# ebeauce/Seismic_BPMF

Measured on AMD Instinct MI355X. Metric: million network-CC-samples/s (matched filter), higher is better.
Workload: dtype f32

## Files before the change

### seismic_bpmf_amd/csrc/mf.hip

```cpp
#include "common.h"
#include "host_call.h"
#include "mf_split_api.h"
#include "mf_full_api.h"
#include <system_error>
#include <thread>
#include <chrono>
#include <vector>
#include <mutex>
#include <utility>
#include <cstring>
#include <algorithm>
#include "../../include/bpmf_hip.h"

#include <cstdlib>

namespace bpmf {

typedef float f32x16 __attribute__((ext_vector_type(16)));


__device__ __forceinline__ int2 mf_lag_range(bool any, long long mv_min, long long mv_max, long long step,
                                             long long L, long long N, long long n_corr, int exclusive_last)
{
    int2 r = make_int2(1, 0);
// ... 302 lines not shown
            mf_stage_rows<MAXR, MF_THREADS>(rd, rs_d, lag0 + mvc, tid);
            const __amdgpu_buffer_rsrc_t rs_t = __builtin_amdgcn_make_buffer_rsrc(
                (void*)(tmpl + ((size_t)t * n_ch + ch) * (size_t)L), 0, L * 4, 0x00020000);
            mf_stage_band<MAXT, MF_THREADS>(rt, rs_t, tid);
        };
        auto write_stage = [&](float* tp, float* dw) {
#pragma unroll
            for (int r = 0; r < MAXR; ++r) {
                const int x = tid + MF_THREADS * r;
                if (x < W) dw[mf_pad(x)] = rd[r];
            }
#pragma unroll
            for (int r = 0; r < MAXT; ++r) {
                const int x = tid + MF_THREADS * r;
                if (x < tp_len) tp[x] = rt[r];
            }
        };
        int4 rec = recs[0];
        int4 rec1 = recs[1];
        int ri = 0;
        if (rec.x >= 0) issue_stage(rec.x, rec.y);
        int buf = 0;
        while (rec.x >= 0) {
            const int ch = rec.x;
            float* tp = smem + buf * buf_floats;
            float* dw = tp + tp_len;
            write_stage(tp, dw);
            __syncthreads();
            const float w = __int_as_float(rec.z);
            const int mvc = rec.y;
            const float et = __int_as_float(rec.w);
            const int4 rec2 = recs[ri + 2];
            const float* edc = e_d + (size_t)ch * (size_t)nwin;
            f32x4 ed[4];
#pragma unroll
            for (int u = 0; u < 4; ++u) {
                const long long lag = lag_w + 256 * u;
                if (wg_inside || (lag + 3 >= rg.x && lag <= rg.y)) {
                    ed[u] = *(const f32x4u*)(edc + lag + mvc);
                } else {
                    ed[u] = (f32x4){0.0f, 0.0f, 0.0f, 0.0f};
                }
            }
            if (rec1.x >= 0) issue_stage(rec1.x, rec1.y);

            f32x4 acc[4];
#pragma unroll
            for (int u = 0; u < 4; ++u) acc[u] = (f32x4){0.0f, 0.0f, 0.0f, 0.0f};
            const int nq = Kpad >> 4;
            const unsigned a_addr = (unsigned)(size_t)(tp + a_base) ;
            const unsigned b_addr = (unsigned)(size_t)(dw + b_base);
            unsigned ap = a_addr, bp = b_addr;
            float sa[4], sb[4][4];
#define MF_LDS_READ(dst, addr, off) \
    asm volatile("ds_read_b32 %0, %1 offset:%2" : "=v"(dst) : "v"(addr), "n"(off))
#define MF_MFMA(slot, u) \
    acc[u] = __builtin_amdgcn_mfma_f32_16x16x4f32(sa[slot], sb[slot][u], acc[u], 0, 0, 0)
#define MF_REQ(slot, aoff, boff)                                    \
    MF_LDS_READ(sa[slot], ap, (aoff));                               \
    MF_LDS_READ(sb[slot][0], bp, (boff));                            \
    MF_LDS_READ(sb[slot][1], bp, (boff) + 1088);                     \
    MF_LDS_READ(sb[slot][2], bp, (boff) + 2176);                     \
    MF_LDS_READ(sb[slot][3], bp, (boff) + 3264)
#define MF_STEP(cur, req, aoff, boff)                                \
    asm volatile("s_waitcnt lgkmcnt(5)" ::: "memory");               \
    __builtin_amdgcn_sched_barrier(0);                               \
    MF_MFMA(cur, 0);                                                 \
    __builtin_amdgcn_sched_barrier(0);                               \
    MF_LDS_READ(sa[req], ap, (aoff));                                \
    __builtin_amdgcn_sched_barrier(0);                               \
    MF_MFMA(cur, 1);                                                 \
    __builtin_amdgcn_sched_barrier(0);                               \
    MF_LDS_READ(sb[req][0], bp, (boff));                             \
    __builtin_amdgcn_sched_barrier(0);                               \
    MF_MFMA(cur, 2);                                                 \
    __builtin_amdgcn_sched_barrier(0);                               \
    MF_LDS_READ(sb[req][1], bp, (boff) + 1088);                      \
    __builtin_amdgcn_sched_barrier(0);                               \
    MF_MFMA(cur, 3);                                                 \
    __builtin_amdgcn_sched_barrier(0);                               \
    MF_LDS_READ(sb[req][2], bp, (boff) + 2176);                      \
    MF_LDS_READ(sb[req][3], bp, (boff) + 3264);                      \
    __builtin_amdgcn_sched_barrier(0)
            __builtin_amdgcn_sched_barrier(0);
            if (prio) __builtin_amdgcn_s_setprio(0);
            MF_REQ(0, 0, 0);
            MF_REQ(1, 16, 16);
            for (int q = 0; q < nq; ++q) {
                MF_STEP(0, 2, 32, 32);
                MF_STEP(1, 3, 48, 48);
                MF_STEP(2, 0, 64, 68);
                MF_STEP(3, 1, 80, 84);
                ap += 64;
                bp += 68;
            }
            asm volatile("s_waitcnt lgkmcnt(0)" ::: "memory");
            __builtin_amdgcn_sched_barrier(0);
            if (prio == 1) __builtin_amdgcn_s_setprio(1);
            else if (prio == 2) __builtin_amdgcn_s_setprio(2);
            else if (prio == 3) __builtin_amdgcn_s_setprio(3);
#undef MF_LDS_READ
#undef MF_MFMA
#undef MF_REQ
#undef MF_STEP

            if (NETWORK_SUM && STEP1 && wg_inside) {
#pragma unroll
                for (int u = 0; u < 4; ++u) {
#pragma unroll
                    for (int r = 0; r < 4; ++r) {
                        const float cc = mf_cc_of<SQRT_NORM>(acc[u][r], et, ed[u][r]);
                        sum[u][r] = __fmaf_rn(w, cc, sum[u][r]);
                    }
                }
            } else {
#pragma unroll
            for (int u = 0; u < 4; ++u) {
#pragma unroll
                for (int r = 0; r < 4; ++r) {
                    const long long lag = lag_w + 256 * u + r;
                    const bool ok = lag >= rg.x && lag <= rg.y && (STEP1 || (unsigned)lag % (unsigned)step == 0);
                    float cc = 0.0f;
                    if (ok) {
                        cc = mf_cc_of<SQRT_NORM>(acc[u][r], et, ed[u][r]);
                        if (!NETWORK_SUM)
                            out[((size_t)t * n_corr + (STEP1 ? lag : (long long)((unsigned)lag / (unsigned)step))) * n_ch + ch] = cc;
                    }
                    if (NETWORK_SUM) sum[u][r] = __fmaf_rn(w, cc, sum[u][r]);
                }
            }
            }
            rec = rec1;
            rec1 = rec2;
            ++ri;
            buf ^= 1;
        }
    }
    if (NETWORK_SUM) {
#pragma unroll
        for (int u = 0; u < 4; ++u) {
            const long long lag = lag_w + 256 * u;
            float* dst = out + (size_t)t * n_corr + lag;
            if (STEP1 && lag + 3 < n_corr) {
                *(f32x4u*)dst = sum[u];
            } else {
#pragma unroll
                for (int r = 0; r < 4; ++r) {
                    const unsigned smp = (unsigned)(lag + r);
                    const long long i = STEP1 ? (long long)smp : (long long)(smp / (unsigned)step);
                    if ((STEP1 || smp % (unsigned)step == 0) && i < n_corr) out[(size_t)t * n_corr + i] = sum[u][r];
                }
            }
        }
    }
}

template <bool SQRT_NORM>
__device__ __forceinline__ int2 mf_fused_prologue(const float* __restrict__ tmpl, const int* __restrict__ mv,
                                                  const float* __restrict__ w, int t, int n_ch, long long step, int L,
                                                  long long N, long long n_corr, int exclusive_last,
                                                  int4* l_rec, int* l_part)
{
    const int tid = threadIdx.x, lane = tid & 63, wv = tid >> 6;
    float wc = 0.0f, nt = 0.0f;
    int m = 0;
    bool used = false;
    if (tid < n_ch) {
        wc = w[(size_t)t * n_ch + tid];
        used = !(wc == 0.0f);
    }
    const bool all_channels = (exclusive_last & 2) != 0;
    if (tid < n_ch && (used || all_channels)) m = mv[(size_t)t * n_ch + tid];
    if (used) {
        const float* x = tmpl + ((size_t)t * n_ch + tid) * (size_t)L;
        float acc = 0.0f;
        int l = 0;
        for (; l + 16 <= L; l += 16) {
            const f32x4u v0 = *(const f32x4u*)(x + l), v1 = *(const f32x4u*)(x + l + 4);
            const f32x4u v2 = *(const f32x4u*)(x + l + 8), v3 = *(const f32x4u*)(x + l + 12);
#pragma unroll
            for (int i = 0; i < 4; ++i) acc = __fmaf_rn(v0[i], v0[i], acc);
#pragma unroll
            for (int i = 0; i < 4; ++i) acc = __fmaf_rn(v1[i], v1[i], acc);
#pragma unroll
            for (int i = 0; i < 4; ++i) acc = __fmaf_rn(v2[i], v2[i], acc);
#pragma unroll
            for (int i = 0; i < 4; ++i) acc = __fmaf_rn(v3[i], v3[i], acc);
        }
        for (; l < L; ++l) acc = __fmaf_rn(x[l], x[l], acc);
        nt = SQRT_NORM ? acc : 1.0f / sqrtf(acc);
    }
    const unsigned long long mask = __ballot(used);
    const int idx = __popcll(mask & ((1ull << lane) - 1ull));
    const bool ranged = used || (all_channels && tid < n_ch);
    int mn = ranged ? m : 0x7fffffff, mx = ranged ? m : (int)0x80000000;
#pragma unroll
    for (int o = 32; o > 0; o >>= 1) {
        mn = min(mn, __shfl_xor(mn, o));
        mx = max(mx, __shfl_xor(mx, o));
    }
    if (lane == 0) {
        l_part[wv] = __popcll(mask);
        l_part[4 + wv] = mn;
        l_part[8 + wv] = mx;
    }
    __syncthreads();
    int base = 0, n_used = 0, mv_min_i = 0x7fffffff, mv_max_i = (int)0x80000000;
#pragma unroll
    for (int i = 0; i < 4; ++i) {
        const int c = l_part[i];
        if (i < wv) base += c;
        n_used += c;
        mv_min_i = min(mv_min_i, l_part[4 + i]);
        mv_max_i = max(mv_max_i, l_part[8 + i]);
    }
    if (used) l_rec[base + idx] = make_int4(tid, m, __float_as_int(wc), __float_as_int(nt));
    if (tid < MF_REC_TERMINATORS) l_rec[n_used + tid] = make_int4(-1, 0, 0, 0);
    __syncthreads();
    return mf_lag_range(n_used > 0, mv_min_i, mv_max_i, step, L, N, n_corr, exclusive_last);
}

#ifdef BPMF_PHASE_CYCLES
__device__ unsigned long long g_mf_phase[8];
#define MF_PHASE_DECL unsigned long long ph_last_ = 0, ph_acc_[4] = {0, 0, 0, 0}; unsigned ph_n_ = 0;
#define MF_PHASE_START() asm volatile("s_memtime %0\n\ts_waitcnt lgkmcnt(0)" : "=s"(ph_last_) :: "memory")
#define MF_PHASE(i)                                                                                \
    do {                                                                                           \
        unsigned long long t_;                                                                     \
        asm volatile("s_memtime %0\n\ts_waitcnt lgkmcnt(0)" : "=s"(t_) :: "memory");              \
        ph_acc_[i] += t_ - ph_last_;                                                               \
        ph_last_ = t_;                                                                             \
    } while (0)
#else
#define MF_PHASE_DECL
#define MF_PHASE_START() do {} while (0)
#define MF_PHASE(i) do {} while (0)
#endif

template <bool NETWORK_SUM, int MAXR, int MAXT, bool STEP1, int NTILE = 4, bool SQRT_NORM = false, bool FUSED = false, bool CSPLIT = false>
__global__ __launch_bounds__(MF_THREADS, 4) void mf_mfma_wave_kernel(
    const float* __restrict__ tmpl, const int4* __restrict__ chan_rec,
    const float* __restrict__ data, const float* __restrict__ e_d,
    const int2* __restrict__ range, int L, long long N, int T, int n_ch, long long n_corr, int step,
    float* __restrict__ out, int n_lag_blocks, int prio, const int* __restrict__ mv,
    const float* __restrict__ wts, int exclusive_last, int lag_block0)
{
    extern __shared__ float smem[];
    const int Kpad = mf_kpad(L);
    const int tp_len = mf_band_len(L);
    static_assert(NTILE == 4 || NTILE == 2 || NTILE == 1, "tiles per wave");
    static_assert(!CSPLIT || (NTILE == 1 && FUSED && NETWORK_SUM && STEP1), "channel split: the tiny-problem variant only");
    constexpr int LAGS_W = 256 * NTILE, LAGS_WG = CSPLIT ? LAGS_W : 4 * LAGS_W;
    constexpr int REC_STRIDE = CSPLIT ? 4 : 1;
    const int Ww = LAGS_W - 16 + Kpad;
    constexpr bool FULLW = NTILE < 4;
    const int Wbuf = FULLW ? 64 * MAXR : Ww;
    const int wave_floats = tp_len + (Wbuf + 2 * (Wbuf >> 4) + 2 + 63) / 64 * 64 + 64;

    const int tid = threadIdx.x;
    const int lane = tid & 63;
    const int wv = __builtin_amdgcn_readfirstlane(tid >> 6);
    const int a = lane & 15;
    const int kq = lane >> 4;

    int t;
    long long lag_block;
    if (!mf_tile_of_block(blockIdx.x, T, n_lag_blocks, t, lag_block)) return;
    lag_block += lag_block0;
    int2 rgi;
    int4* l_rec = nullptr;
    if constexpr (FUSED) {
        int* l_part = (int*)(smem + 4 * wave_floats + 64);
        l_rec = (int4*)(l_part + 16);
        const int2 r = mf_fused_prologue<SQRT_NORM>(tmpl, mv, wts, t, n_ch, (long long)step, L, N, n_corr, exclusive_last,
                                                    l_rec, l_part);
        rgi = make_int2(__builtin_amdgcn_readfirstlane(r.x), __builtin_amdgcn_readfirstlane(r.y));
    } else {
        rgi = range[t];
    }
    float* exch = nullptr;
    int n_used = 0;
    if constexpr (CSPLIT) {
        const int* l_part = (const int*)(smem + 4 * wave_floats + 64);
        n_used = l_part[0] + l_part[1] + l_part[2] + l_part[3];
        exch = (float*)(l_rec + n_ch + MF_REC_TERMINATORS);
    }
    const long long lag0 = lag_block * LAGS_WG + (CSPLIT ? 0 : (long long)wv * LAGS_W);
    const int2 rg = make_int2(rgi.x * step, rgi.y * step);
    const long long nwin = N - L + 1;

    f32x4 sum[NTILE];
#pragma unroll
    for (int u = 0; u < NTILE; ++u) sum[u] = (f32x4){0.0f, 0.0f, 0.0f, 0.0f};

    const bool wave_valid = rg.x <= rg.y && !(lag0 > rg.y || lag0 + LAGS_W - 1 < rg.x);
    const bool wave_inside = lag0 >= rg.x && lag0 + LAGS_W - 1 <= rg.y;
    const long long lag_w = lag0 + 16 * a + 4 * kq;
    MF_PHASE_DECL

    if (wave_valid) {
        float* tp = smem + wv * wave_floats;
        float* dw = tp + tp_len;
        const int a_base = 15 - a + kq;
        const int b_base = 18 * a + kq;
        const int4* __restrict__ recs = FUSED ? nullptr : chan_rec + (size_t)t * (n_ch + 2);
        auto ld_rec = [&](int i) -> int4 {
            if constexpr (FUSED) {
                const int4 v = l_rec[i];
                return make_int4(__builtin_amdgcn_readfirstlane(v.x), __builtin_amdgcn_readfirstlane(v.y),
                                 __builtin_amdgcn_readfirstlane(v.z), __builtin_amdgcn_readfirstlane(v.w));
            } else {
                return recs[i];
            }
        };

        float rd[MAXR], rt[MAXT];
        auto issue_stage = [&](int ch, int mvc) {
            const __amdgpu_buffer_rsrc_t rs_d = __builtin_amdgcn_make_buffer_rsrc(
                (void*)(data + (size_t)ch * (size_t)N), 0, (int)(N * 4), 0x00020000);
            mf_stage_rows<MAXR, 64>(rd, rs_d, lag0 + mvc, lane);
            const __amdgpu_buffer_rsrc_t rs_t = __builtin_amdgcn_make_buffer_rsrc(
                (void*)(tmpl + ((size_t)t * n_ch + ch) * (size_t)L), 0, L * 4, 0x00020000);
            mf_stage_band<MAXT, 64>(rt, rs_t, lane);
        };
        const int rd_chunks = (Ww + 63) >> 6, rt_chunks = (tp_len + 63) >> 6;
        auto write_stage = [&]() {
            if constexpr (FULLW) {
#pragma unroll
                for (int r = 0; r < MAXT; ++r) tp[lane + 64 * r] = rt[r];
#pragma unroll
                for (int r = 0; r < MAXR; ++r) {
                    const int x = lane + 64 * r;
                    dw[x + 2 * (x >> 4)] = rd[r];
                }
                return;
            }
#define MF_WT(r) case (r) + 1: if constexpr ((r) < MAXT) tp[lane + 64 * ((r) < MAXT ? (r) : 0)] = rt[(r) < MAXT ? (r) : 0]; [[fallthrough]];
            switch (rt_chunks) {
                MF_WT(4) MF_WT(3) MF_WT(2) MF_WT(1) MF_WT(0)
                default: break;
            }
#undef MF_WT
#define MF_WD(r) case (r) + 1: if constexpr ((r) < MAXR) { const int x = lane + 64 * (r); dw[x + 2 * (x >> 4)] = rd[(r) < MAXR ? (r) : 0]; } [[fallthrough]];
            switch (rd_chunks) {
                MF_WD(19) MF_WD(18) MF_WD(17) MF_WD(16) MF_WD(15) MF_WD(14) MF_WD(13) MF_WD(12) MF_WD(11) MF_WD(10)
                MF_WD(9) MF_WD(8) MF_WD(7) MF_WD(6) MF_WD(5) MF_WD(4) MF_WD(3) MF_WD(2) MF_WD(1) MF_WD(0)
                default: break;
            }
#undef MF_WD
        };

        int4 rec = ld_rec(CSPLIT ? wv : 0);
        int4 rec1 = ld_rec(CSPLIT ? wv + REC_STRIDE : 1);
        int ri = CSPLIT ? wv : 0;
        if (rec.x >= 0) issue_stage(rec.x, rec.y);
        MF_PHASE_START();
        while (rec.x >= 0) {
            const int ch = rec.x;
            write_stage();
            MF_PHASE(0);
            const float w = __int_as_float(rec.z);
            const int mvc = rec.y;
            const float et = __int_as_float(rec.w);
            const int4 rec2 = ld_rec(ri + 2 * REC_STRIDE);
            const float* edc = e_d + (size_t)ch * (size_t)nwin;
            f32x4 ed[NTILE];
            if (wave_inside) {
#pragma unroll
                for (int u = 0; u < NTILE; ++u) ed[u] = *(const f32x4u*)(edc + lag_w + 256 * u + mvc);
            } else {
#pragma unroll
                for (int u = 0; u < NTILE; ++u) {
                    const long long lag = lag_w + 256 * u;
                    if (lag + 3 >= rg.x && lag <= rg.y) {
                        ed[u] = *(const f32x4u*)(edc + lag + mvc);
                    } else {
                        ed[u] = (f32x4){0.0f, 0.0f, 0.0f, 0.0f};
                    }
                }
            }
            if (rec1.x >= 0) issue_stage(rec1.x, rec1.y);
            MF_PHASE(1);

            f32x4 acc[NTILE];
#pragma unroll
            for (int u = 0; u < NTILE; ++u) acc[u] = (f32x4){0.0f, 0.0f, 0.0f, 0.0f};
            const int nq = Kpad >> 4;
            unsigned ap = (unsigned)(size_t)(tp + a_base), bp = (unsigned)(size_t)(dw + b_base);
            float sa[4], sb[4][NTILE];
#define MF_LDS_READ(dst, addr, off) \
    asm volatile("ds_read_b32 %0, %1 offset:%2" : "=v"(dst) : "v"(addr), "n"(off))
#define MF_MFMA(slot, u) \
    acc[u] = __builtin_amdgcn_mfma_f32_16x16x4f32(sa[slot], sb[slot][u], acc[u], 0, 0, 0)
#define MF_REQ(slot, aoff, boff)                                                    \
    MF_LDS_READ(sa[slot], ap, (aoff));                                               \
    MF_LDS_READ(sb[slot][0], bp, (boff));                                            \
    if constexpr (NTILE > 1) MF_LDS_READ(sb[slot][1 % NTILE], bp, (boff) + 1152);    \
    if constexpr (NTILE > 2) MF_LDS_READ(sb[slot][2 % NTILE], bp, (boff) + 2304);    \
    if constexpr (NTILE > 2) MF_LDS_READ(sb[slot][3 % NTILE], bp, (boff) + 3456)
#define MF_STEP(cur, req, aoff, boff)                                                \
    asm volatile("s_waitcnt lgkmcnt(%0)" :: "n"(NTILE + 1) : "memory");              \
    __builtin_amdgcn_sched_barrier(0);                                               \
    MF_MFMA(cur, 0);                                                                 \
    __builtin_amdgcn_sched_barrier(0);                                               \
    MF_LDS_READ(sa[req], ap, (aoff));                                                \
    __builtin_amdgcn_sched_barrier(0);                                               \
    if constexpr (NTILE > 1) { MF_MFMA(cur, 1 % NTILE); __builtin_amdgcn_sched_barrier(0); } \
    MF_LDS_READ(sb[req][0], bp, (boff));                                             \
    __builtin_amdgcn_sched_barrier(0);                                               \
    if constexpr (NTILE > 2) { MF_MFMA(cur, 2 % NTILE); __builtin_amdgcn_sched_barrier(0); } \
    if constexpr (NTILE > 1) { MF_LDS_READ(sb[req][1 % NTILE], bp, (boff) + 1152); __builtin_amdgcn_sched_barrier(0); } \
    if constexpr (NTILE > 2) { MF_MFMA(cur, 3 % NTILE); __builtin_amdgcn_sched_barrier(0); } \
    if constexpr (NTILE > 2) { MF_LDS_READ(sb[req][2 % NTILE], bp, (boff) + 2304); MF_LDS_READ(sb[req][3 % NTILE], bp, (boff) + 3456); } \
    __builtin_amdgcn_sched_barrier(0)
            __builtin_amdgcn_sched_barrier(0);
            if (prio) __builtin_amdgcn_s_setprio(0);
            MF_REQ(0, 0, 0);
            MF_REQ(1, 16, 16);
            for (int q = 0; q < nq; ++q) {
                MF_STEP(0, 2, 32, 32);
                MF_STEP(1, 3, 48, 48);
                MF_STEP(2, 0, 64, 72);
                MF_STEP(3, 1, 80, 88);
                ap += 64;
                bp += 72;
            }
            asm volatile("s_waitcnt lgkmcnt(0)" ::: "memory");
            __builtin_amdgcn_sched_barrier(0);
            if (prio == 1) __builtin_amdgcn_s_setprio(1);
            else if (prio == 2) __builtin_amdgcn_s_setprio(2);
            else if (prio == 3) __builtin_amdgcn_s_setprio(3);
#undef MF_LDS_READ
#undef MF_MFMA
#undef MF_REQ
#undef MF_STEP
            MF_PHASE(2);
            if constexpr (CSPLIT) {
                f32x4 c4;
#pragma unroll
                for (int r = 0; r < 4; ++r) {
                    const long long lag = lag_w + r;
                    const bool ok = wave_inside || (lag >= rg.x && lag <= rg.y);
                    c4[r] = ok ? mf_cc_of<SQRT_NORM>(acc[0][r], et, ed[0][r]) : 0.0f;
                }
                *(f32x4*)(exch + ri * 256 + 16 * a + 4 * kq) = c4;
            } else if (NETWORK_SUM && STEP1 && wave_inside) {
#pragma unroll
                for (int u = 0; u < NTILE; ++u) {
#pragma unroll
                    for (int r = 0; r < 4; ++r) {
                        const float cc = mf_cc_of<SQRT_NORM>(acc[u][r], et, ed[u][r]);
                        sum[u][r] = __fmaf_rn(w, cc, sum[u][r]);
                    }
                }
            } else {
#pragma unroll
            for (int u = 0; u < NTILE; ++u) {
#pragma unroll
                for (int r = 0; r < 4; ++r) {
                    const long long lag = lag_w + 256 * u + r;
                    const bool ok = lag >= rg.x && lag <= rg.y && (STEP1 || (unsigned)lag % (unsigned)step == 0);
                    float cc = 0.0f;
                    if (ok) {
                        cc = mf_cc_of<SQRT_NORM>(acc[u][r], et, ed[u][r]);
                        if (!NETWORK_SUM)
                            out[((size_t)t * n_corr + (STEP1 ? lag : (long long)((unsigned)lag / (unsigned)step))) * n_ch + ch] = cc;
                    }
                    if (NETWORK_SUM) sum[u][r] = __fmaf_rn(w, cc, sum[u][r]);
                }
            }
            }
            rec = rec1;
            rec1 = rec2;
            ri += REC_STRIDE;
            MF_PHASE(3);
#ifdef BPMF_PHASE_CYCLES
            ++ph_n_;
#endif
        }
    }
    if constexpr (CSPLIT) {
        __syncthreads();
        const long long lag = lag0 + tid;
        float s = 0.0f;
        if (wave_valid) {
            for (int i = 0; i < n_used; ++i) s = __fmaf_rn(__int_as_float(l_rec[i].z), exch[i * 256 + tid], s);
        }
        if (lag < n_corr) out[(size_t)t * n_corr + lag] = s;
    } else if (NETWORK_SUM) {
#pragma unroll
        for (int u = 0; u < NTILE; ++u) {
            const long long lag = lag_w + 256 * u;
            float* dst = out + (size_t)t * n_corr + lag;
            if (STEP1 && lag + 3 < n_corr) {
                *(f32x4u*)dst = sum[u];
            } else {
#pragma unroll
                for (int r = 0; r < 4; ++r) {
                    const unsigned smp = (unsigned)(lag + r);
                    const long long i = STEP1 ? (long long)smp : (long long)(smp / (unsigned)step);
                    if ((STEP1 || smp % (unsigned)step == 0) && i < n_corr) out[(size_t)t * n_corr + i] = sum[u][r];
                }
            }
        }
    }
#ifdef BPMF_PHASE_CYCLES
    if (lane == 0 && ph_n_) {
        for (int i = 0; i < 4; ++i) atomicAdd(&g_mf_phase[i], ph_acc_[i]);
        atomicAdd(&g_mf_phase[4], (unsigned long long)ph_n_);
        atomicAdd(&g_mf_phase[5], 1ull);
    }
#endif
}

template <bool NETWORK_SUM, bool SQRT_NORM = false>
__global__ __launch_bounds__(256) void mf_direct_kernel(
    const float* __restrict__ tmpl, const int* __restrict__ mv, const float* __restrict__ wgt,
    const float* __restrict__ data, const float* __restrict__ e_t,
    const float* __restrict__ e_d, const int2* __restrict__ range, long long step, int L,
    long long N, int n_ch, long long n_corr, float* __restrict__ out,
    const double* __restrict__ cs_local = nullptr, const double* __restrict__ cs_off = nullptr, long long nq = 0)
{
    const long long i = (long long)blockIdx.x * blockDim.x + threadIdx.x;
    const int t = blockIdx.y;
    if (i >= n_corr) return;
    const int2 rg = range[t];
    const bool ok = i >= rg.x && i <= rg.y;
    const long long nwin = N - L + 1;
    float sum = 0.0f;
    if (ok) {
        for (int ch = 0; ch < n_ch; ++ch) {
            const float w = wgt[(size_t)t * n_ch + ch];
            if (w == 0.0f) continue;
            const long long j = i * step + mv[(size_t)t * n_ch + ch];
            const float* tp = tmpl + ((size_t)t * n_ch + ch) * (size_t)L;
            const float* d = data + (size_t)ch * (size_t)N + j;
            float num = 0.0f;
            for (int l = 0; l < L; ++l) num = __fmaf_rn(tp[l], d[l], num);
            float cc = 0.0f;
            if constexpr (SQRT_NORM) {
                float et = 0.0f;
                for (int l = 0; l < L; ++l) et = __fmaf_rn(tp[l], tp[l], et);
                const double* lo = cs_local + (size_t)ch * (size_t)N;
                const double* of = cs_off + (size_t)ch * (size_t)nq;
                const long long nh = j + L - 1;
                const double hi = of[nh / CSUM_CHUNK] + lo[nh];
                const double low = j > 0 ? of[(j - 1) / CSUM_CHUNK] + lo[j - 1] : 0.0;
                const float den2 = et * (float)(hi - low);
                if (den2 > 1.0e-6f) cc = num / sqrtf(den2);
            } else {
                const float nrm = e_t[(size_t)t * n_ch + ch] * e_d[(size_t)ch * nwin + j];
                if (nrm < MAX_NORM) cc = num * nrm;
            }
            if (NETWORK_SUM)
                sum = __fmaf_rn(w, cc, sum);
            else
                out[((size_t)t * n_corr + i) * n_ch + ch] = cc;
        }
    }
    if (NETWORK_SUM) out[(size_t)t * n_corr + i] = sum;
}

struct MfWorkspace {
    double* local;
    double* tot;
    double* off;
    float* e_d;
    float* e_t;
    int2* range;
    int4* chan_rec;
    void* sp_day;
    void* sp_batch;
    size_t bytes;
};

static MfWorkspace mf_carve(void* base, size_t L, size_t N, size_t T, size_t n_ch)
{
    MfWorkspace ws;
    const size_t nq = (N + CSUM_CHUNK - 1) / CSUM_CHUNK;
    const size_t nwin = N >= L ? N - L + 1 : 0;
    char* p = (char*)base;
    size_t o = 0;
    ws.local = (double*)(p + o); o += align_up(n_ch * N * sizeof(double), 256);
    ws.tot = (double*)(p + o);   o += align_up(n_ch * nq * sizeof(double), 256);
    ws.off = (double*)(p + o);   o += align_up(n_ch * nq * sizeof(double), 256);
    o += 256;
    ws.e_d = (float*)(p + o);    o += align_up(n_ch * nwin * sizeof(float) + 64, 256);
    const bool split16 = option(OPT_MF_SPLIT16) != 0;
    ws.sp_day = nullptr;
    ws.sp_batch = nullptr;
    if (split16) { ws.sp_day = p + o; o += align_up(sp::day_region_bytes(N, n_ch), 256); }
    ws.e_t = (float*)(p + o);    o += align_up(T * n_ch * sizeof(float), 256);
    ws.range = (int2*)(p + o);   o += align_up(T * sizeof(int2), 256);
    ws.chan_rec = (int4*)(p + o); o += align_up(T * (n_ch + 2) * sizeof(int4), 256);
    if (split16) { ws.sp_batch = p + o; o += align_up(sp::batch_region_bytes(T, n_ch, L), 256); }
    ws.bytes = o;
    return ws;
}

struct MfFullWorkspace {
    MfWorkspace ws;
    full::DayRegion day;
    float* tprime;
};

static MfFullWorkspace mf_carve_full(void* base, size_t L, size_t N, size_t T, size_t n_ch)
{
    MfFullWorkspace f;
    MfWorkspace& ws = f.ws;
    const size_t nq = (N + CSUM_CHUNK - 1) / CSUM_CHUNK;
    const size_t nwin = N >= L ? N - L + 1 : 0;
    char* p = (char*)base;
    size_t o = 0;
    ws.local = (double*)(p + o); o += align_up(n_ch * N * sizeof(double), 256);
    ws.tot = (double*)(p + o);   o += align_up(n_ch * nq * sizeof(double), 256);
    ws.off = (double*)(p + o);   o += align_up(n_ch * nq * sizeof(double), 256);
    o += 256;
    ws.e_d = (float*)(p + o);    o += align_up(n_ch * nwin * sizeof(float) + 64, 256);
    ws.sp_day = nullptr;
    ws.sp_batch = nullptr;
    f.day = full::carve_day(p + o, N, n_ch); o += f.day.bytes;
    ws.e_t = (float*)(p + o);    o += align_up(T * n_ch * sizeof(float), 256);
    ws.range = (int2*)(p + o);   o += align_up(T * sizeof(int2), 256);
    ws.chan_rec = (int4*)(p + o); o += align_up(T * (n_ch + 2) * sizeof(int4), 256);
    f.tprime = (float*)(p + o);  o += full::batch_region_bytes(T, n_ch, L);
    ws.bytes = o;
    return f;
}

static int mf_check_sizes(size_t step, size_t L, size_t N, size_t T, size_t S, size_t C,
                          size_t n_corr)
{
    if (step == 0 || L == 0 || T == 0 || S == 0 || C == 0) {
        set_error("matched filter: zero-sized dimension (step=%zu L=%zu T=%zu S=%zu C=%zu)", step,
                  L, T, S, C);
        return -1;
    }
    if (N < L) {
        set_error("matched filter: data (N=%zu) shorter than the templates (L=%zu)", N, L);
        return -1;
    }
    if (n_corr != (N - L) / step + 1) {
        set_error("matched filter: n_corr=%zu but (N-L)/step+1=%zu", n_corr, (N - L) / step + 1);
        return -1;
    }
    if (N > 0x7fffffffull || T * S * C > 0x7fffffffull || L > 0x7fffffffull) {
        set_error("matched filter: dimension exceeds the int32 index range");
        return -1;
    }
    return 0;
}

struct MfLaunch {
    long long off_lo = 0, off_hi = -1;
    bool first_piece = true;
};

struct SplitDay { const void* data; size_t N, n_ch; };
struct DayRegistry {
    std::mutex mutex;
    std::vector<std::pair<const void*, SplitDay>> days;
    void note(const void* ws_base, const void* data, size_t N, size_t n_ch, bool listed)
    {
        std::lock_guard<std::mutex> g(mutex);
        for (size_t i = 0; i < days.size(); ++i)
            if (days[i].first == ws_base) { days.erase(days.begin() + i); break; }
        if (listed) {
            if (days.size() >= 64) days.erase(days.begin());
            days.push_back({ws_base, {data, N, n_ch}});
        }
    }
    int known(const void* ws_base, const void* data, size_t N, size_t n_ch)
    {
        std::lock_guard<std::mutex> g(mutex);
        for (auto& e : days)
            if (e.first == ws_base) return e.second.data == data && e.second.N == N && e.second.n_ch == n_ch ? 1 : -1;
        return 0;
    }
};
static DayRegistry g_split_days, g_full_days;
static void split_day_note(const void* ws_base, const void* data, size_t N, size_t n_ch, bool with_split)
{
    g_split_days.note(ws_base, data, N, n_ch, with_split);
}
static bool split_day_known(const void* ws_base, const void* data, size_t N, size_t n_ch)
{
    return g_split_days.known(ws_base, data, N, n_ch) == 1;
}
static void full_day_note(const void* ws_base, const void* data, size_t N, size_t n_ch, bool is_full)
{
    g_full_days.note(ws_base, data, N, n_ch, is_full);
}
static int full_day_known(const void* ws_base, const void* data, size_t N, size_t n_ch)
{
    return g_full_days.known(ws_base, data, N, n_ch);
}

static const char* mf_full_refused_option()
{
    if (option(OPT_MF_COMPAT_SQRT_NORM) != 0) return "mf.compat_sqrt_norm";
    if (option(OPT_MF_COMPAT_SEQUENTIAL_CSUM) != 0) return "mf.compat_sequential_csum";
    return nullptr;
}

enum MfFamily { MF_DIRECT = 0, MF_WORKGROUP = 1, MF_WAVE = 2, MF_SPLIT16 = 3 };
enum MfRefusal { MF_ACCEPTED = 0, MF_GRID_TOO_LARGE = 1, MF_TOO_MANY_TEMPLATES = 2 };
static const char* const MF_REFUSAL_TEXT[] = {"", "grid too large", "generic kernel supports at most 65535 templates per call"};

struct MfVariant {
    int family, refusal;
    int maxr, maxt;
    int ntile;
    bool fused, csplit;
    bool sqrt_norm, step1, prologue;
    size_t lags_wg, lds, grid;
};

constexpr int MF_WAVE_MAXT = 5;
constexpr int mf_wave_maxr(int ntile) { return ntile == 4 ? 20 : (ntile == 2 ? 12 : 8); }
static size_t mf_grid(size_t T, size_t n_blocks) { return 8 * ((T * n_blocks + 7) / 8); }

static MfVariant mf_choose(size_t step, size_t L, size_t N, size_t T, size_t n_ch, size_t n_corr, int network_sum,
                           int flags, bool ranged)
{
    MfVariant v = {};
    v.sqrt_norm = option(OPT_MF_COMPAT_SQRT_NORM) != 0;
    v.step1 = step == 1;
    v.prologue = true;
    const size_t n_offsets = (n_corr - 1) * step + 1;
    const size_t n_lag_blocks = (n_offsets + MF_LAGS_PER_WG - 1) / MF_LAGS_PER_WG;
    const int need_r = (mf_window_len((int)L) + MF_THREADS - 1) / MF_THREADS;
    const int need_t = (mf_band_len((int)L) + MF_THREADS - 1) / MF_THREADS;
    const bool mfma = step <= (size_t)option(OPT_MF_MAX_MFMA_STEP) && !(flags & BPMF_MF_FORCE_DIRECT) && need_r <= 24 &&
                      need_t <= 9 && T * (n_lag_blocks + 8) < 0x7fffffffull && N < ((size_t)1 << 30) - 8192;
    if (!mfma) {
        v.family = MF_DIRECT;
        v.lags_wg = 256;
        v.grid = (n_corr + 255) / 256 * T;
        if (T > 65535) v.refusal = MF_TOO_MANY_TEMPLATES;
        return v;
    }
    constexpr size_t SP_MIN_BLOCKS = 128;
    const size_t sp_blocks = (n_offsets + sp::LAGS_PER_WG - 1) / sp::LAGS_PER_WG;
    const bool sp_small = option(OPT_MF_SPLIT16) == 1 && T * sp_blocks < SP_MIN_BLOCKS;
    if (option(OPT_MF_SPLIT16) != 0 && sp::usable(L, N) && !sp_small && !(flags & BPMF_MF_NORMALIZE_FULL)) {
        v.family = MF_SPLIT16;
        v.lags_wg = sp::LAGS_PER_WG;
        v.grid = mf_grid(T, sp_blocks);
// ... 508 lines not shown
```

Baseline: 4376.

## Use phase-split LDS data layout with paired ds_read for 4-tile MFMA loop

```diff
diff --git a/seismic_bpmf_amd/csrc/mf.hip b/seismic_bpmf_amd/csrc/mf.hip
--- a/seismic_bpmf_amd/csrc/mf.hip
+++ b/seismic_bpmf_amd/csrc/mf.hip
@@ -628,7 +628,10 @@
         float* tp = smem + wv * wave_floats;
         float* dw = tp + tp_len;
         const int a_base = 15 - a + kq;
-        const int b_base = 18 * a + kq;
+        const int rd_chunks = (Ww + 63) >> 6, rt_chunks = (tp_len + 63) >> 6;
+        const int PH = 16 * (rd_chunks | 1) + 2;
+        const int b_base = NTILE == 4 ? kq * PH + 4 * a : 18 * a + kq;
+        float* const dws = dw + (lane & 3) * PH + (lane >> 2);
         const int4* __restrict__ recs = FUSED ? nullptr : chan_rec + (size_t)t * (n_ch + 2);
         auto ld_rec = [&](int i) -> int4 {
             if constexpr (FUSED) {
@@ -649,7 +652,6 @@
                 (void*)(tmpl + ((size_t)t * n_ch + ch) * (size_t)L), 0, L * 4, 0x00020000);
             mf_stage_band<MAXT, 64>(rt, rs_t, lane);
         };
-        const int rd_chunks = (Ww + 63) >> 6, rt_chunks = (tp_len + 63) >> 6;
         auto write_stage = [&]() {
             if constexpr (FULLW) {
 #pragma unroll
@@ -667,7 +669,7 @@
                 default: break;
             }
 #undef MF_WT
-#define MF_WD(r) case (r) + 1: if constexpr ((r) < MAXR) { const int x = lane + 64 * (r); dw[x + 2 * (x >> 4)] = rd[(r) < MAXR ? (r) : 0]; } [[fallthrough]];
+#define MF_WD(r) case (r) + 1: if constexpr ((r) < MAXR) dws[16 * (r)] = rd[(r) < MAXR ? (r) : 0]; [[fallthrough]];
             switch (rd_chunks) {
                 MF_WD(19) MF_WD(18) MF_WD(17) MF_WD(16) MF_WD(15) MF_WD(14) MF_WD(13) MF_WD(12) MF_WD(11) MF_WD(10)
                 MF_WD(9) MF_WD(8) MF_WD(7) MF_WD(6) MF_WD(5) MF_WD(4) MF_WD(3) MF_WD(2) MF_WD(1) MF_WD(0)
@@ -713,6 +715,46 @@
             for (int u = 0; u < NTILE; ++u) acc[u] = (f32x4){0.0f, 0.0f, 0.0f, 0.0f};
             const int nq = Kpad >> 4;
             unsigned ap = (unsigned)(size_t)(tp + a_base), bp = (unsigned)(size_t)(dw + b_base);
+            if constexpr (NTILE == 4) {
+            typedef float f32x2 __attribute__((ext_vector_type(2)));
+            f32x2 pa[2], pb[2][4];
+#define MF_RD_A(slot, o0) \
+    asm volatile("ds_read2_b32 %0, %1 offset0:%2 offset1:%3" : "=v"(pa[slot]) : "v"(ap), "n"(o0), "n"((o0) + 4))
+#define MF_RD_B(slot, u, off) \
+    asm volatile("ds_read_b64 %0, %1 offset:%2" : "=v"(pb[slot][u]) : "v"(bp), "n"((off) + 256 * (u)))
+#define MF_MFMA2(slot, u, j) \
+    acc[u] = __builtin_amdgcn_mfma_f32_16x16x4f32(pa[slot][j], pb[slot][u][j], acc[u], 0, 0, 0)
+#define MF_SB __builtin_amdgcn_sched_barrier(0)
+#define MF_PAIR(cur, ao, bo)                                                         \
+    asm volatile("s_waitcnt lgkmcnt(2)" ::: "memory"); MF_SB;                        \
+    MF_MFMA2(cur, 0, 0); MF_SB; MF_RD_A((cur) ^ 1, ao); MF_SB;                       \
+    MF_MFMA2(cur, 1, 0); MF_SB;                                                      \
+    asm volatile("s_waitcnt lgkmcnt(1)" ::: "memory"); MF_SB;                        \
+    MF_MFMA2(cur, 2, 0); MF_SB; MF_RD_B((cur) ^ 1, 0, bo); MF_SB;                    \
+    MF_MFMA2(cur, 3, 0); MF_SB; MF_RD_B((cur) ^ 1, 1, bo); MF_SB;                    \
+    MF_MFMA2(cur, 0, 1); MF_SB; MF_RD_B((cur) ^ 1, 2, bo); MF_SB;                    \
+    MF_MFMA2(cur, 1, 1); MF_SB; MF_RD_B((cur) ^ 1, 3, bo); MF_SB;                    \
+    MF_MFMA2(cur, 2, 1); MF_SB;                                                      \
+    MF_MFMA2(cur, 3, 1); MF_SB
+            MF_SB;
+            if (prio) __builtin_amdgcn_s_setprio(0);
+            MF_RD_A(0, 0);
+            MF_RD_B(0, 0, 0); MF_RD_B(0, 1, 0); MF_RD_B(0, 2, 0); MF_RD_B(0, 3, 0);
+            int q = nq;
+            do {
+                MF_PAIR(0, 8, 8);
+                MF_PAIR(1, 16, 16);
+                ap += 64;
+                bp += 16;
+            } while (--q > 0);
+            asm volatile("s_waitcnt lgkmcnt(0)" ::: "memory");
+            MF_SB;
+#undef MF_RD_A
+#undef MF_RD_B
+#undef MF_MFMA2
+#undef MF_PAIR
+#undef MF_SB
+            } else {
             float sa[4], sb[4][NTILE];
 #define MF_LDS_READ(dst, addr, off) \
     asm volatile("ds_read_b32 %0, %1 offset:%2" : "=v"(dst) : "v"(addr), "n"(off))
@@ -753,13 +795,14 @@
             }
             asm volatile("s_waitcnt lgkmcnt(0)" ::: "memory");
             __builtin_amdgcn_sched_barrier(0);
-            if (prio == 1) __builtin_amdgcn_s_setprio(1);
-            else if (prio == 2) __builtin_amdgcn_s_setprio(2);
-            else if (prio == 3) __builtin_amdgcn_s_setprio(3);
 #undef MF_LDS_READ
 #undef MF_MFMA
 #undef MF_REQ
 #undef MF_STEP
+            }
+            if (prio == 1) __builtin_amdgcn_s_setprio(1);
+            else if (prio == 2) __builtin_amdgcn_s_setprio(2);
+            else if (prio == 3) __builtin_amdgcn_s_setprio(3);
             MF_PHASE(2);
             if constexpr (CSPLIT) {
                 f32x4 c4;
@@ -770,6 +813,29 @@
                     c4[r] = ok ? mf_cc_of<SQRT_NORM>(acc[0][r], et, ed[0][r]) : 0.0f;
                 }
                 *(f32x4*)(exch + ri * 256 + 16 * a + 4 * kq) = c4;
+            } else if constexpr (NETWORK_SUM && STEP1 && NTILE == 4) {
+                if (wave_inside) {
+#pragma unroll
+                    for (int u = 0; u < NTILE; ++u) {
+#pragma unroll
+                        for (int r = 0; r < 4; ++r) acc[u][r] = mf_cc_of<SQRT_NORM>(acc[u][r], et, ed[u][r]);
+                    }
+                } else {
+#pragma unroll
+                    for (int u = 0; u < NTILE; ++u) {
+#pragma unroll
+                        for (int r = 0; r < 4; ++r) {
+                            const long long lag = lag_w + 256 * u + r;
+                            const bool ok = lag >= rg.x && lag <= rg.y;
+                            acc[u][r] = ok ? mf_cc_of<SQRT_NORM>(acc[u][r], et, ed[u][r]) : 0.0f;
+                        }
+                    }
+                }
+#pragma unroll
+                for (int u = 0; u < NTILE; ++u) {
+#pragma unroll
+                    for (int r = 0; r < 4; ++r) sum[u][r] = __fmaf_rn(w, acc[u][r], sum[u][r]);
+                }
             } else if (NETWORK_SUM && STEP1 && wave_inside) {
 #pragma unroll
                 for (int u = 0; u < NTILE; ++u) {
```

After: 4439 (median of 6 runs). 1.4% higher.
